# Runbook-Agent/RunbookAI

Hardware: NVIDIA H100
Metric: knn_queries_per_sec (higher is better)
Workload: dtype bf16

## Files before the change

### runbookai_b200/csrc/rbk_epilogue.cuh

```cuda
#pragma once
#include "rbk_internal.h"
#include "rbk_ptx.cuh"

namespace rbk {

struct FilterState {
  float thr;
  float inv_q;
  float qn;
  int tb;
  int mb_cache;
  int cnt;
  bool valid;
  bool nohist;
  unsigned long long* list;
  unsigned int* hist_q;
  int* maxbin_q;
};

__device__ __forceinline__ int score_bin(float a) {
  const int b = static_cast<int>((a + 1.0f) * (kHistBins * 0.5f));
  return min(max(b, 0), kHistBins - 1);
}
__device__ __forceinline__ float bin_edge_raw(int b, float qn) {
  const float edge = static_cast<float>(b) * (2.0f / kHistBins) - 1.0f - 1e-6f;
  const float r = edge * qn;
  return r - fabsf(r) * 1e-6f;
}

__device__ __forceinline__ void filter_init(FilterState& s, bool valid, float thr_init, float inv_q,
                                            unsigned long long* list, unsigned int* hist_q, int* maxbin_q) {
  s.valid = valid && thr_init < INFINITY;
  s.thr = s.valid ? thr_init : INFINITY;
  s.inv_q = s.valid ? inv_q : 0.f;
  s.qn = s.valid ? 1.0f / inv_q : 0.f;
  s.tb = (s.valid && thr_init > -INFINITY) ? score_bin(thr_init * inv_q) : -1;
  s.mb_cache = -1;
  s.nohist = false;
  s.cnt = 0;
  s.list = list;
  s.hist_q = hist_q;
  s.maxbin_q = maxbin_q;
}

static __device__ __noinline__ unsigned long long histogram_walk(const unsigned int* hist_q, int mb, int tb, float qn,
                                                                  int kprime) {
  const uint4* h4 = reinterpret_cast<const uint4*>(hist_q);
  const int g_lo = (tb + 1) >> 2;
  unsigned cum = 0;
  for (int g_hi = mb >> 2; g_hi >= g_lo; g_hi -= 4) {
    uint4 w[4];
#pragma unroll
    for (int u = 0; u < 4; ++u) w[u] = (g_hi - u >= g_lo) ? __ldcg(h4 + g_hi - u) : make_uint4(0u, 0u, 0u, 0u);
#pragma unroll
    for (int u = 0; u < 4; ++u) {
      const int g = g_hi - u;
      const unsigned c[4] = {w[u].x, w[u].y, w[u].z, w[u].w};
#pragma unroll
      for (int j = 3; j >= 0; --j) {
        const int b = g * 4 + j;
        if (g >= g_lo && b <= mb && b > tb) {
          cum += c[j];
          if (cum >= static_cast<unsigned>(kprime))
            return (static_cast<unsigned long long>(b + 1) << 32) | __float_as_uint(bin_edge_raw(b, qn));
        }
      }
    }
  }
  return 0ull;
}
__device__ __forceinline__ bool filter_refresh(FilterState& s, int kprime) {
  if (!s.valid) return false;
  const int mb = __ldcg(s.maxbin_q);
  if (mb <= s.tb) return false;
  const unsigned long long r = histogram_walk(s.hist_q, mb, s.tb, s.qn, kprime);
  if (r == 0ull) return false;
  s.tb = static_cast<int>(r >> 32) - 1;
  s.thr = fmaxf(s.thr, __uint_as_float(static_cast<uint32_t>(r)));
  return true;
}

__device__ __forceinline__ bool refresh_due(int it) {
  return it != 0 && (it < 8 || (it < 64 && (it & 7) == 0) || (it & 31) == 0);
}
__device__ __forceinline__ bool publish_due(int it) {
  return it != 0 && (it < 16 || (it < 64 && (it & 1) == 0) || (it & 7) == 0);
}
__device__ __forceinline__ void publish_threshold(FilterState& s, unsigned int* gthr_q, int kprime) {
  if (!s.valid) return;
  s.tb = max(s.tb, score_bin(s.thr * s.inv_q) - 1);
  filter_refresh(s, kprime);
  if (s.thr > -INFINITY) atomicMax(gthr_q, f32_ordered(s.thr));
}
__device__ __forceinline__ void adopt_threshold(FilterState& s, unsigned int ordered) {
  s.thr = fmaxf(s.thr, f32_from_ordered(ordered));
}

__device__ __forceinline__ void hist_add(FilterState& s, float t) {
  const int b = score_bin(t * s.inv_q);
  atomicAdd(s.hist_q + b, 1u);
  if (b > s.mb_cache) {
    atomicMax(s.maxbin_q, b);
    s.mb_cache = b;
  }
}

__device__ __forceinline__ void filter_append(FilterState& s, float t, uint32_t row) {
  s.list[s.cnt] = pack_key(t, row);
  ++s.cnt;
  if (s.nohist) return;
  hist_add(s, t);
}

__device__ __forceinline__ void seed_chunk(FilterState& s, const uint32_t (&v)[32], bool whole_tile, float& acc1,
                                           float& acc2) {
  float m1 = -INFINITY, m2 = -INFINITY;
#pragma unroll
  for (int j = 0; j < 8; ++j) {
    const float a0 = __uint_as_float(v[4 * j + 0]);
    const float a1 = __uint_as_float(v[4 * j + 1]);
    const float a2 = __uint_as_float(v[4 * j + 2]);
    const float a3 = __uint_as_float(v[4 * j + 3]);
    const float x = fmaxf(fmaxf(fmaxf(a0, a1), fmaxf(a2, a3)), -INFINITY);
    m2 = fmaxf(m2, fminf(m1, x));
    m1 = fmaxf(m1, x);
  }
  if (whole_tile) {
    const float lo = fmaxf(fminf(acc1, m1), fmaxf(acc2, m2));
    acc1 = fmaxf(acc1, m1);
    acc2 = lo;
    return;
  }
  if (m1 > s.thr) hist_add(s, m1);
  if (m2 > s.thr) hist_add(s, m2);
}

__device__ __forceinline__ void filter_chunk(FilterState& s, const uint32_t (&v)[32], uint32_t row_base) {
  float g[8];
  float m = -INFINITY;
#pragma unroll
  for (int j = 0; j < 8; ++j) {
    const float a0 = __uint_as_float(v[4 * j + 0]);
    const float a1 = __uint_as_float(v[4 * j + 1]);
    const float a2 = __uint_as_float(v[4 * j + 2]);
    const float a3 = __uint_as_float(v[4 * j + 3]);
    g[j] = fmaxf(fmaxf(a0, a1), fmaxf(a2, a3));
    m = fmaxf(m, g[j]);
  }
  if (m > s.thr) {
#pragma unroll
    for (int j = 0; j < 8; ++j) {
      if (g[j] > s.thr) {
#pragma unroll
        for (int e = 0; e < 4; ++e) {
          const float t = __uint_as_float(v[4 * j + e]);
          if (t > s.thr) filter_append(s, t, row_base + 4 * j + e);
        }
      }
    }
  }
}

__device__ __forceinline__ unsigned long long umax64(unsigned long long a, unsigned long long b) {
  return a > b ? a : b;
}
__device__ __forceinline__ unsigned long long umin64(unsigned long long a, unsigned long long b) {
  return a < b ? a : b;
}

static __device__ __noinline__ unsigned long long warp_compact(unsigned long long* list, int cnt, int kprime, int lane) {
  constexpr uint32_t kFullMask = 0xFFFFFFFFu;
  unsigned long long k[8];
#pragma unroll
  for (int j = 0; j < 8; ++j) {
    const int idx = j * 32 + lane;
    k[j] = idx < cnt ? __ldcg(list + idx) : 0ull;
  }
#pragma unroll
  for (int k2 = 2; k2 <= 256; k2 <<= 1) {
#pragma unroll
    for (int st = k2 >> 1; st > 0; st >>= 1) {
      if (st >= 32) {
        const int js = st >> 5;
#pragma unroll
        for (int j = 0; j < 8; ++j) {
          if ((j & js) == 0) {
            const int i = j * 32 + lane;
            const bool desc = (i & k2) == 0;
            const unsigned long long a = k[j], b = k[j | js];
            const unsigned long long hi = umax64(a, b), lo = umin64(a, b);
            k[j] = desc ? hi : lo;
            k[j | js] = desc ? lo : hi;
          }
        }
      } else {
#pragma unroll
        for (int j = 0; j < 8; ++j) {
          const int i = j * 32 + lane;
          const unsigned long long other = __shfl_xor_sync(kFullMask, k[j], st);
          const bool lower = (lane & st) == 0;
          const bool desc = (i & k2) == 0;
          k[j] = (lower == desc) ? umax64(k[j], other) : umin64(k[j], other);
        }
      }
    }
  }
  const int keep = cnt < kprime ? cnt : kprime;
#pragma unroll
  for (int j = 0; j < 8; ++j) {
    const int idx = j * 32 + lane;
    if (idx < keep) list[idx] = k[j];
  }
  const int e = kprime - 1;
  unsigned long long sel = 0ull;
#pragma unroll
  for (int j = 0; j < 8; ++j)
    if (j == (e >> 5)) sel = k[j];
  const unsigned long long kth = __shfl_sync(kFullMask, sel, e & 31);
  const float new_thr = cnt >= kprime ? key_score(kth) : -INFINITY;
  __syncwarp();
  return (static_cast<unsigned long long>(__float_as_uint(new_thr)) << 32) | static_cast<unsigned>(keep);
}

__device__ __forceinline__ void filter_compact_if_needed(FilterState& s, int kprime, int lane, int room = 32) {
  constexpr uint32_t kFullMask = 0xFFFFFFFFu;
  __syncwarp();
  unsigned need = __ballot_sync(kFullMask, s.cnt > kListCap - room);
  while (need) {
    const int src = __ffs(need) - 1;
    need &= need - 1;
    unsigned long long* l = reinterpret_cast<unsigned long long*>(
        __shfl_sync(kFullMask, reinterpret_cast<unsigned long long>(s.list), src));
    const int c = __shfl_sync(kFullMask, s.cnt, src);
    const unsigned long long r = warp_compact(l, c, kprime, lane);
    if (lane == src) {
      s.thr = fmaxf(s.thr, __uint_as_float(static_cast<uint32_t>(r >> 32)));
      s.cnt = static_cast<int>(static_cast<uint32_t>(r));
    }
  }
}


constexpr int kScorePitch = kBlockN + 4;

__device__ __forceinline__ void load_chunk(const float* src, uint32_t (&v)[32]) {
  const float4* s4 = reinterpret_cast<const float4*>(src);
#pragma unroll
  for (int j = 0; j < 8; ++j) {
    const float4 w = s4[j];
    v[4 * j + 0] = __float_as_uint(w.x);
    v[4 * j + 1] = __float_as_uint(w.y);
    v[4 * j + 2] = __float_as_uint(w.z);
    v[4 * j + 3] = __float_as_uint(w.w);
  }
}

struct StageHeader {
  unsigned long long mask;
  int last;
};
struct StageLink {
  const float* rows;
  const StageHeader* hdr;
  unsigned long long* full;
  unsigned long long* empty;
  volatile float* thr_pub;
};
__device__ __forceinline__ const float* stage_round(const StageLink& l, uint32_t phase, int qw, bool& last) {
  mbar_wait(smem_u32(l.full), phase);
  const unsigned long long mask = l.hdr->mask;
  last = l.hdr->last != 0;
  if (((mask >> qw) & 1ull) == 0ull) return nullptr;
  return l.rows + __popcll(mask & ((1ull << qw) - 1ull)) * kScorePitch;
}

__device__ __forceinline__ void run_epilogue(const ScanParams& p, const StageLink& sl, int qb, int r, int t0, int t1,
                                             int et, int lane) {
  const int q = qb * kBlockM + et;
  const bool q_valid = q < p.B;
  const size_t list_id = static_cast<size_t>(qb * p.R + r) * kBlockM + et;
  FilterState fs;
  filter_init(fs, q_valid, q_valid ? p.thr_init[q] : INFINITY, q_valid ? p.inv_norm_q[q] : 0.f,
              p.cand + list_id * static_cast<size_t>(kListCap),
              p.hist + static_cast<size_t>(q_valid ? q : 0) * kHistBins, p.maxbin + (q_valid ? q : 0));
  const int n_iter = t1 - t0;
  const int qw = et & 63;
  uint32_t phase = 0;
  float pub = -INFINITY;
  unsigned int* gthr_q = p.gthr + (q_valid ? q : 0);
  unsigned int ngt = 0u;
  for (int it = 0; it < n_iter; ++it) {
    const int tile = t0 + it;
    const int row0 = tile * kBlockN;
    adopt_threshold(fs, ngt);
    ngt = __ldcg(gthr_q);
    if (publish_due(it) && r == it % p.R) publish_threshold(fs, gthr_q, p.kprime);
    if (fs.thr > pub) *sl.thr_pub = pub = fs.thr;
    for (bool last = false; !last; phase ^= 1u) {
      const float* srow = stage_round(sl, phase, qw, last);
      const bool staged = srow != nullptr;
      if (__any_sync(0xFFFFFFFFu, staged)) {
        auto process = [&](uint32_t (&v)[32], int chunk) {
          filter_chunk(fs, v, static_cast<uint32_t>(row0 + chunk * 32));
          if (p.dbg_scores != nullptr && q_valid) {
#pragma unroll
            for (int j = 0; j < 32; ++j) {
              const int row = row0 + chunk * 32 + j;
              if (row < p.n_rows) p.dbg_scores[static_cast<size_t>(q) * p.n_rows + row] = __uint_as_float(v[j]);
            }
          }
        };
        uint32_t va[32], vb[32];
        if (it == 0) {
          float sa1 = -INFINITY, sa2 = -INFINITY;
          if (staged) {
#pragma unroll 1
            for (int chunk = 0; chunk < kBlockN / 32; ++chunk) {
              load_chunk(srow + chunk * 32, va);
              seed_chunk(fs, va, false, sa1, sa2);
            }
          }
          const int tries = (p.R * 16 >= 2 * p.kprime) ? 6 : 1;
          for (int t = 0; t < tries; ++t) {
            const bool found = staged && filter_refresh(fs, p.kprime);
            if (__all_sync(0xFFFFFFFFu, found || !fs.valid || !staged)) break;
            if (t + 1 < tries) __nanosleep(400);
          }
          if (staged && fs.valid && fs.thr > -INFINITY) atomicMax(gthr_q, f32_ordered(fs.thr));
          fs.nohist = staged;
        }
#pragma unroll 1
        for (int c2 = 0; c2 < kBlockN / 64; ++c2) {
          if (staged) {
            load_chunk(srow + (2 * c2) * 32, va);
            load_chunk(srow + (2 * c2 + 1) * 32, vb);
            process(va, 2 * c2);
            process(vb, 2 * c2 + 1);
          }
          filter_compact_if_needed(fs, p.kprime, lane, 64);
          if (it == 0 && staged && fs.valid && fs.thr == -INFINITY) adopt_threshold(fs, __ldcg(gthr_q));
        }
        fs.nohist = false;
      }
      mbar_arrive(smem_u32(sl.empty));
    }
    if (fs.thr > pub) *sl.thr_pub = pub = fs.thr;
  }
  p.cand_cnt[list_id] = fs.cnt;
}


__device__ __forceinline__ float count_floor_raw(int b, float qn, float delta) {
  const float edge = static_cast<float>(b) * (2.0f / kHistBins) - 1.0f - delta;
  const float r = edge * qn;
  return r - fabsf(r) * 1e-6f;
}

__device__ __forceinline__ void run_count_epilogue(const LargeScanParams& p, const StageLink& sl, int qb, int t0,
                                                   int t1, int et) {
  const int q = qb * kBlockM + et;
  const bool q_valid = q < p.B;
  FilterState fs;
  filter_init(fs, q_valid, q_valid ? p.thr_init[q] : INFINITY, q_valid ? p.inv_norm_q[q] : 0.f, nullptr,
              p.hist + static_cast<size_t>(q_valid ? q : 0) * kHistBins, p.maxbin + (q_valid ? q : 0));
  const float delta = q_valid ? static_cast<float>(2.0 * p.q_eps[q]) + 2.0f / kHistBins : 0.f;
  const int n_iter = t1 - t0;
  const int qw = et & 63;
  uint32_t phase = 0;
  float pub = -INFINITY;
  for (int it = 0; it < n_iter; ++it) {
    if (fs.valid && refresh_due(it)) {
      const int mb = __ldcg(fs.maxbin_q);
      if (mb > fs.tb) {
        const unsigned long long w = histogram_walk(fs.hist_q, mb, fs.tb, fs.qn, p.kprime);
        if (w != 0ull) {
          fs.tb = static_cast<int>(w >> 32) - 1;
          fs.thr = fmaxf(fs.thr, count_floor_raw(fs.tb, fs.qn, delta));
        }
      }
    }
    if (fs.thr > pub) *sl.thr_pub = pub = fs.thr;
    for (bool last = false; !last; phase ^= 1u) {
      const float* srow = stage_round(sl, phase, qw, last);
      if (srow != nullptr) {
#pragma unroll 1
        for (int chunk = 0; chunk < kBlockN / 32; ++chunk) {
          uint32_t v[32];
          load_chunk(srow + chunk * 32, v);
          float g[8];
          float m = -INFINITY;
#pragma unroll
          for (int j = 0; j < 8; ++j) {
            const float a0 = __uint_as_float(v[4 * j + 0]);
            const float a1 = __uint_as_float(v[4 * j + 1]);
            const float a2 = __uint_as_float(v[4 * j + 2]);
            const float a3 = __uint_as_float(v[4 * j + 3]);
            g[j] = fmaxf(fmaxf(a0, a1), fmaxf(a2, a3));
            m = fmaxf(m, g[j]);
          }
          if (m >= fs.thr) {
#pragma unroll
            for (int j = 0; j < 8; ++j) {
              if (g[j] >= fs.thr) {
#pragma unroll
                for (int e = 0; e < 4; ++e) {
                  const float a = __uint_as_float(v[4 * j + e]);
                  if (a >= fs.thr) hist_add(fs, a);
                }
              }
            }
          }
        }
      }
      mbar_arrive(smem_u32(sl.empty));
    }
  }
}

__device__ __forceinline__ void run_emit_epilogue(const LargeScanParams& p, const StageLink& sl, int qb, int t0,
                                                  int t1, int et) {
  const int q = qb * kBlockM + et;
  const bool q_valid = q < p.B;
  const float theta = q_valid ? p.thr_init[q] : INFINITY;
  const bool live = q_valid && theta < INFINITY;
  const long long seg = live ? p.emit_off[q] : 0;
  const int cap = live ? p.emit_cap[q] : 0;
  const int n_iter = t1 - t0;
  const int qw = et & 63;
  uint32_t phase = 0;
  *sl.thr_pub = theta;
  for (int it = 0; it < n_iter; ++it) {
    const int row0 = (t0 + it) * kBlockN;
    for (bool last = false; !last; phase ^= 1u) {
      const float* srow = stage_round(sl, phase, qw, last);
      if (srow != nullptr) {
#pragma unroll 1
        for (int chunk = 0; chunk < kBlockN / 32; ++chunk) {
          uint32_t v[32];
          load_chunk(srow + chunk * 32, v);
          uint32_t hits = 0u;
#pragma unroll
          for (int j = 0; j < 32; ++j) hits |= (__uint_as_float(v[j]) >= theta ? 1u : 0u) << j;
          if (hits != 0u && live) {
            int pos = atomicAdd(p.emit_cnt + q, __popc(hits));
            const int row_base = row0 + chunk * 32;
            while (hits != 0u) {
              const int j = __ffs(hits) - 1;
              hits &= hits - 1u;
              if (pos < cap) p.emit_rows[seg + pos] = row_base + j;
              ++pos;
            }
          }
        }
      }
      mbar_arrive(smem_u32(sl.empty));
    }
  }
}

static_assert(kMaxSubBatch / kBlockM <= 32, "one lane per query block");
__device__ __forceinline__ void lockstep_pace(volatile int* prog, int QB, int qb, int it, int max_lead, int lane) {
  if (QB <= 1 || (it & 1) != 0) return;
  if (lane == 0) prog[qb] = it;
  const bool peer = lane < QB && lane != qb;
  const int floor = it - max_lead;
  bool behind = peer && prog[lane] < floor;
  const long long w0 = clock64();
  while (__any_sync(0xFFFFFFFFu, behind)) {
    __nanosleep(200);
    if (__shfl_sync(0xFFFFFFFFu, clock64() - w0, 0) > (1ll << 24)) break;
    behind = peer && prog[lane] < floor;
  }
}

}
```

### runbookai_b200/csrc/rbk_ptx.cuh

```cuda
#pragma once
#include <cuda_runtime.h>
#include <stdint.h>

namespace rbk {

__device__ __forceinline__ uint32_t smem_u32(const void* p) {
  return static_cast<uint32_t>(__cvta_generic_to_shared(p));
}

__device__ __forceinline__ void mbar_init(uint32_t bar, uint32_t count) {
  asm volatile("mbarrier.init.shared::cta.b64 [%0], %1;" ::"r"(bar), "r"(count) : "memory");
}
__device__ __forceinline__ void fence_barrier_init() {
  asm volatile("fence.mbarrier_init.release.cluster;" ::: "memory");
}
__device__ __forceinline__ void mbar_arrive(uint32_t bar) {
  asm volatile("mbarrier.arrive.shared::cta.b64 _, [%0];" ::"r"(bar) : "memory");
}
__device__ __forceinline__ void mbar_arrive_expect_tx(uint32_t bar, uint32_t bytes) {
  asm volatile("mbarrier.arrive.expect_tx.shared::cta.b64 _, [%0], %1;" ::"r"(bar), "r"(bytes) : "memory");
}
__device__ __forceinline__ bool mbar_try_wait(uint32_t bar, uint32_t parity) {
  uint32_t ok;
  asm volatile(
      "{\n\t.reg .pred p;\n\t"
      "mbarrier.try_wait.parity.shared::cta.b64 p, [%1], %2;\n\t"
      "selp.u32 %0, 1, 0, p;\n\t}"
      : "=r"(ok)
      : "r"(bar), "r"(parity)
      : "memory");
  return ok != 0;
}
__device__ __forceinline__ void mbar_wait(uint32_t bar, uint32_t parity) {
  if (mbar_try_wait(bar, parity)) return;
  const long long t0 = clock64();
  uint32_t spins = 0;
  while (!mbar_try_wait(bar, parity)) {
    if (((++spins) & 0x3FFu) == 0 && (clock64() - t0) > (1ll << 31)) __trap();
  }
}

__device__ __forceinline__ void tma_prefetch_desc(const void* tmap) {
  asm volatile("prefetch.tensormap [%0];" ::"l"(reinterpret_cast<uint64_t>(tmap)) : "memory");
}
__device__ __forceinline__ void tma_load_2d(uint32_t smem_dst, const void* tmap, uint32_t bar, int32_t crd0,
                                            int32_t crd1) {
  asm volatile(
      "cp.async.bulk.tensor.2d.shared::cluster.global.mbarrier::complete_tx::bytes [%0], [%1, {%3, %4}], [%2];"
      :
      : "r"(smem_dst), "l"(reinterpret_cast<uint64_t>(tmap)), "r"(bar), "r"(crd0), "r"(crd1)
      : "memory");
}

__device__ __forceinline__ void bulk_load(uint32_t smem_dst, const void* src, uint32_t bytes, uint32_t bar) {
  asm volatile("cp.async.bulk.shared::cluster.global.mbarrier::complete_tx::bytes [%0], [%1], %2, [%3];"
               :
               : "r"(smem_dst), "l"(reinterpret_cast<uint64_t>(src)), "r"(bytes), "r"(bar)
               : "memory");
}

__device__ __forceinline__ void wgmma_fence() { asm volatile("wgmma.fence.sync.aligned;" ::: "memory"); }
__device__ __forceinline__ void wgmma_commit() { asm volatile("wgmma.commit_group.sync.aligned;" ::: "memory"); }
template <int N>
__device__ __forceinline__ void wgmma_wait(float (&d)[128]) {
  asm volatile("wgmma.wait_group.sync.aligned %0;" ::"n"(N) : "memory");
#pragma unroll
  for (int i = 0; i < 128; ++i) asm volatile("" : "+f"(d[i])::"memory");
}

__device__ __forceinline__ uint64_t make_sw128_kmajor_desc(uint32_t smem_addr) {
  uint64_t d = 0;
  d |= static_cast<uint64_t>((smem_addr & 0x3FFFFu) >> 4);
  d |= static_cast<uint64_t>(1) << 16;
  d |= static_cast<uint64_t>(1024 >> 4) << 32;
  d |= static_cast<uint64_t>(1) << 62;
  return d;
}

#define RBK_WGMMA_D128                                                                                              \
  "{%0, %1, %2, %3, %4, %5, %6, %7, %8, %9, %10, %11, %12, %13, %14, %15, "                                         \
  "%16, %17, %18, %19, %20, %21, %22, %23, %24, %25, %26, %27, %28, %29, %30, %31, "                                \
  "%32, %33, %34, %35, %36, %37, %38, %39, %40, %41, %42, %43, %44, %45, %46, %47, "                                \
  "%48, %49, %50, %51, %52, %53, %54, %55, %56, %57, %58, %59, %60, %61, %62, %63, "                                \
  "%64, %65, %66, %67, %68, %69, %70, %71, %72, %73, %74, %75, %76, %77, %78, %79, "                                \
  "%80, %81, %82, %83, %84, %85, %86, %87, %88, %89, %90, %91, %92, %93, %94, %95, "                                \
  "%96, %97, %98, %99, %100, %101, %102, %103, %104, %105, %106, %107, %108, %109, %110, %111, "                    \
  "%112, %113, %114, %115, %116, %117, %118, %119, %120, %121, %122, %123, %124, %125, %126, %127}"
#define RBK_WGMMA_D128_OUT(d)                                                                                         \
  "+f"(d[0]), "+f"(d[1]), "+f"(d[2]), "+f"(d[3]), "+f"(d[4]), "+f"(d[5]), "+f"(d[6]), "+f"(d[7]), "+f"(d[8]),      \
      "+f"(d[9]), "+f"(d[10]), "+f"(d[11]), "+f"(d[12]), "+f"(d[13]), "+f"(d[14]), "+f"(d[15]), "+f"(d[16]),         \
      "+f"(d[17]), "+f"(d[18]), "+f"(d[19]), "+f"(d[20]), "+f"(d[21]), "+f"(d[22]), "+f"(d[23]), "+f"(d[24]),        \
      "+f"(d[25]), "+f"(d[26]), "+f"(d[27]), "+f"(d[28]), "+f"(d[29]), "+f"(d[30]), "+f"(d[31]), "+f"(d[32]),        \
      "+f"(d[33]), "+f"(d[34]), "+f"(d[35]), "+f"(d[36]), "+f"(d[37]), "+f"(d[38]), "+f"(d[39]), "+f"(d[40]),        \
      "+f"(d[41]), "+f"(d[42]), "+f"(d[43]), "+f"(d[44]), "+f"(d[45]), "+f"(d[46]), "+f"(d[47]), "+f"(d[48]),        \
      "+f"(d[49]), "+f"(d[50]), "+f"(d[51]), "+f"(d[52]), "+f"(d[53]), "+f"(d[54]), "+f"(d[55]), "+f"(d[56]),        \
      "+f"(d[57]), "+f"(d[58]), "+f"(d[59]), "+f"(d[60]), "+f"(d[61]), "+f"(d[62]), "+f"(d[63]), "+f"(d[64]),        \
      "+f"(d[65]), "+f"(d[66]), "+f"(d[67]), "+f"(d[68]), "+f"(d[69]), "+f"(d[70]), "+f"(d[71]), "+f"(d[72]),        \
      "+f"(d[73]), "+f"(d[74]), "+f"(d[75]), "+f"(d[76]), "+f"(d[77]), "+f"(d[78]), "+f"(d[79]), "+f"(d[80]),        \
      "+f"(d[81]), "+f"(d[82]), "+f"(d[83]), "+f"(d[84]), "+f"(d[85]), "+f"(d[86]), "+f"(d[87]), "+f"(d[88]),        \
      "+f"(d[89]), "+f"(d[90]), "+f"(d[91]), "+f"(d[92]), "+f"(d[93]), "+f"(d[94]), "+f"(d[95]), "+f"(d[96]),        \
      "+f"(d[97]), "+f"(d[98]), "+f"(d[99]), "+f"(d[100]), "+f"(d[101]), "+f"(d[102]), "+f"(d[103]), "+f"(d[104]),   \
      "+f"(d[105]), "+f"(d[106]), "+f"(d[107]), "+f"(d[108]), "+f"(d[109]), "+f"(d[110]), "+f"(d[111]),              \
      "+f"(d[112]), "+f"(d[113]), "+f"(d[114]), "+f"(d[115]), "+f"(d[116]), "+f"(d[117]), "+f"(d[118]),              \
      "+f"(d[119]), "+f"(d[120]), "+f"(d[121]), "+f"(d[122]), "+f"(d[123]), "+f"(d[124]), "+f"(d[125]),              \
      "+f"(d[126]), "+f"(d[127])

__device__ __forceinline__ void wgmma_m64n256k16_bf16(float (&d)[128], uint64_t desc_a, uint64_t desc_b,
                                                      uint32_t accumulate) {
  asm volatile(
      "{\n\t.reg .pred p;\n\t"
      "setp.ne.b32 p, %130, 0;\n\t"
      "wgmma.mma_async.sync.aligned.m64n256k16.f32.bf16.bf16 " RBK_WGMMA_D128 ", %128, %129, p, 1, 1, 0, 0;\n\t}"
      : RBK_WGMMA_D128_OUT(d)
      : "l"(desc_a), "l"(desc_b), "r"(accumulate));
}
__device__ __forceinline__ void wgmma_m64n256k16_f16(float (&d)[128], uint64_t desc_a, uint64_t desc_b,
                                                     uint32_t accumulate) {
  asm volatile(
      "{\n\t.reg .pred p;\n\t"
      "setp.ne.b32 p, %130, 0;\n\t"
      "wgmma.mma_async.sync.aligned.m64n256k16.f32.f16.f16 " RBK_WGMMA_D128 ", %128, %129, p, 1, 1, 0, 0;\n\t}"
      : RBK_WGMMA_D128_OUT(d)
      : "l"(desc_a), "l"(desc_b), "r"(accumulate));
}

__device__ __forceinline__ bool elect_one() {
  uint32_t pred;
  asm volatile(
      "{\n\t.reg .pred p;\n\t"
      "elect.sync _|p, 0xFFFFFFFF;\n\t"
      "selp.u32 %0, 1, 0, p;\n\t}"
      : "=r"(pred));
  return pred != 0;
}

template <uint32_t N>
__device__ __forceinline__ void setmaxnreg_dec() {
  asm volatile("setmaxnreg.dec.sync.aligned.u32 %0;" ::"n"(N));
}
template <uint32_t N>
__device__ __forceinline__ void setmaxnreg_inc() {
  asm volatile("setmaxnreg.inc.sync.aligned.u32 %0;" ::"n"(N));
}
__device__ __forceinline__ void named_bar_sync(uint32_t id, uint32_t nthreads) {
  asm volatile("bar.sync %0, %1;" ::"r"(id), "r"(nthreads) : "memory");
}

__device__ __forceinline__ uint32_t f32_ordered(float f) {
  uint32_t u = __float_as_uint(f);
  return (u & 0x80000000u) ? ~u : (u | 0x80000000u);
}
__device__ __forceinline__ float f32_from_ordered(uint32_t o) {
  uint32_t u = (o & 0x80000000u) ? (o & 0x7FFFFFFFu) : ~o;
  return __uint_as_float(u);
}
__device__ __forceinline__ uint64_t pack_key(float score, uint32_t row) {
  return (static_cast<uint64_t>(f32_ordered(score)) << 32) | static_cast<uint64_t>(0xFFFFFFFFu - row);
}
__device__ __forceinline__ uint32_t key_row(uint64_t k) { return 0xFFFFFFFFu - static_cast<uint32_t>(k); }
__device__ __forceinline__ float key_score(uint64_t k) { return f32_from_ordered(static_cast<uint32_t>(k >> 32)); }

}
```

### runbookai_b200/csrc/rbk_scan.cu

```cuda
#define RBK_SCAN_F16 0
#include "rbk_scan_kernel.cuh"

namespace rbk {

cudaError_t launch_scan(const CUtensorMap& tmap_q, const CUtensorMap& tmap_c, const ScanParams& p,
                        cudaStream_t stream) {
  return launch_scan_mode<0>(tmap_q, tmap_c, p, stream);
}

cudaError_t launch_scan_large(const CUtensorMap& tmap_q, const CUtensorMap& tmap_c, const LargeScanParams& p,
                              LargeScanMode mode, cudaStream_t stream) {
  if (mode == kScanCount) return launch_scan_mode<kScanCount>(tmap_q, tmap_c, p, stream);
  return launch_scan_mode<kScanEmit>(tmap_q, tmap_c, p, stream);
}

}

#ifdef RBK_SCAN_CYCLE_STATS
extern "C" int rbk_scan_cycle_stats(unsigned long long* out) {
  constexpr int n = 3 * 2 * (rbk::kCycBuckets + 2);
  static const unsigned long long zero[n] = {};
  if (cudaDeviceSynchronize() != cudaSuccess ||
      cudaMemcpyFromSymbol(out, rbk::g_cycle_stats, sizeof(zero)) != cudaSuccess ||
      cudaMemcpyToSymbol(rbk::g_cycle_stats, zero, sizeof(zero)) != cudaSuccess)
    return -1;
  return n;
}
#endif
```

### runbookai_b200/csrc/rbk_scan_kernel.cuh

```cuda
#pragma once
#ifndef RBK_SCAN_F16
#error "define RBK_SCAN_F16 (0: bf16 operands, 1: fp16 operands) before including rbk_scan_kernel.cuh"
#endif
#if defined(RBK_SCAN_CYCLE_STATS) && !RBK_SCAN_F16
#define RBK_SCAN_PROBE 1
#else
#define RBK_SCAN_PROBE 0
#endif

#include "rbk_epilogue.cuh"
#include "rbk_internal.h"
#include "rbk_ptx.cuh"

namespace rbk {

namespace {

constexpr int kABytes = kBlockM * kBlockK * 2;
constexpr int kBBytes = kBlockN * kBlockK * 2;
constexpr int kStageBytes = kABytes + kBBytes;
constexpr int kMmaThreads = 256;
constexpr int kStagingBytes = 2 * kStageRows * kScorePitch * 4;
static_assert(kScanThreads == 128 + kMmaThreads, "warp roles");
static_assert(2 * kStageRows <= kBlockM, "a round never holds more rows than a warpgroup has queries");

struct SmemTail {
  float invc[2][2][kBlockN];
  float thr[kBlockM];
  StageHeader hdr[2];
  uint16_t wmask[2][2][4];
  unsigned long long full[kStages];
  unsigned long long empty[kStages];
  unsigned long long invc_full[2][2];
  unsigned long long st_full[2];
  unsigned long long st_empty[2];
};
constexpr size_t kScanSmemBytes = static_cast<size_t>(kStages) * kStageBytes + kStagingBytes + sizeof(SmemTail) + 1024;
static_assert(kScanSmemBytes <= 227 * 1024, "scan kernel shared memory exceeds the sm_90 per-block limit");

__device__ __forceinline__ void scan_mma(float (&d)[128], uint64_t desc_a, uint64_t desc_b, uint32_t accumulate) {
#if RBK_SCAN_F16
  wgmma_m64n256k16_f16(d, desc_a, desc_b, accumulate);
#else
  wgmma_m64n256k16_bf16(d, desc_a, desc_b, accumulate);
#endif
}

__device__ __forceinline__ void store_row(float* dst, const float (&d)[128], int h, int lane) {
  float* r = dst + 2 * (lane & 3);
#pragma unroll
  for (int j = 0; j < kBlockN / 8; ++j)
    *reinterpret_cast<float2*>(r + 8 * j) = make_float2(d[4 * j + 2 * h], d[4 * j + 2 * h + 1]);
}

__device__ __forceinline__ uint32_t quad_bits(uint32_t b) {
  b &= 0x11111111u;
  b = (b | (b >> 3)) & 0x03030303u;
  b = (b | (b >> 6)) & 0x000F000Fu;
  return (b | (b >> 12)) & 0xFFu;
}

enum CycleBucket { kCycFull, kCycMma, kCycHandoff, kCycPace, kCycTileEnd, kCycBuckets };
#if RBK_SCAN_PROBE
__device__ unsigned long long g_cycle_stats[3][2][kCycBuckets + 2];
__device__ __forceinline__ uint32_t sm_clock() {
  uint32_t c;
  asm volatile("mov.u32 %0, %%clock;" : "=r"(c)::"memory");
  return c;
}
struct CycleProbe {
  uint32_t t = 0, c[kCycBuckets] = {};
  __device__ __forceinline__ void mark() { t = sm_clock(); }
  __device__ __forceinline__ void lap(int b) {
    const uint32_t n = sm_clock();
    c[b] += n - t;
    t = n;
  }
  __device__ __forceinline__ void add_since(int b, uint32_t t0) { c[b] += sm_clock() - t0; }
  __device__ __forceinline__ static uint32_t now() { return sm_clock(); }
};
#else
struct CycleProbe {
  __device__ __forceinline__ void mark() {}
  __device__ __forceinline__ void lap(int) {}
  __device__ __forceinline__ void add_since(int, uint32_t) {}
  __device__ __forceinline__ static uint32_t now() { return 0u; }
};
#endif

template <int kMode, typename P>
__global__ void __launch_bounds__(kScanThreads, 1)
scan_kernel(const __grid_constant__ CUtensorMap tmap_q, const __grid_constant__ CUtensorMap tmap_c,
            const P p) {
  extern __shared__ uint8_t smem_raw[];
  const uint32_t raw_addr = smem_u32(smem_raw);
  uint8_t* smem = smem_raw + ((1024u - (raw_addr & 1023u)) & 1023u);
  float* staging = reinterpret_cast<float*>(smem + kStages * kStageBytes);
  SmemTail* tail = reinterpret_cast<SmemTail*>(smem + kStages * kStageBytes + kStagingBytes);
  const uint32_t smem_base = smem_u32(smem);

  const int warp = threadIdx.x >> 5;
  const int lane = threadIdx.x & 31;
  const int wgroup = warp >> 2;
  const int qb = blockIdx.x % p.QB;
  const int r = blockIdx.x / p.QB;
  const int t0 = static_cast<int>(static_cast<long long>(p.n_tiles) * r / p.R);
  const int t1 = static_cast<int>(static_cast<long long>(p.n_tiles) * (r + 1) / p.R);
  const int n_ks = p.dpad / kBlockK;

  if (threadIdx.x < kBlockM) tail->thr[threadIdx.x] = -INFINITY;
  if (threadIdx.x == 128) {
    tma_prefetch_desc(&tmap_q);
    tma_prefetch_desc(&tmap_c);
    for (int s = 0; s < kStages; ++s) {
      mbar_init(smem_u32(&tail->full[s]), 1);
      mbar_init(smem_u32(&tail->empty[s]), 2);
    }
    for (int w = 0; w < 2; ++w) {
      mbar_init(smem_u32(&tail->invc_full[w][0]), 1);
      mbar_init(smem_u32(&tail->invc_full[w][1]), 1);
      mbar_init(smem_u32(&tail->st_full[w]), 128);
      mbar_init(smem_u32(&tail->st_empty[w]), 64);
    }
    fence_barrier_init();
  }
  __syncthreads();

  constexpr uint32_t kEpiRegs = 152, kMmaRegs = 176;
  static_assert(128 * kEpiRegs + kMmaThreads * kMmaRegs <= kScanThreads * 168, "register split");
  if (wgroup == 0) {
    setmaxnreg_dec<kEpiRegs>();
    const int h = threadIdx.x >> 6;
    const StageLink sl{staging + h * kStageRows * kScorePitch, &tail->hdr[h], &tail->st_full[h], &tail->st_empty[h],
                       &tail->thr[threadIdx.x]};
    if constexpr (kMode == 0)
      run_epilogue(p, sl, qb, r, t0, t1, threadIdx.x, lane);
    else if constexpr (kMode == kScanCount)
      run_count_epilogue(p, sl, qb, t0, t1, threadIdx.x);
    else
      run_emit_epilogue(p, sl, qb, t0, t1, threadIdx.x);
    return;
  }

  setmaxnreg_inc<kMmaRegs>();
  const int wg = wgroup - 1;
  const bool leader = (threadIdx.x & 127) == 0;
  const bool producer = warp == 4;
  const int n_iter = t1 - t0;
  const int n_steps = n_iter * n_ks;
  volatile int* prog = p.progress + r * p.QB;
  CycleProbe probe;
  auto issue = [&](int j) {
    if (j >= n_steps) return;
    const int s = j % kStages;
    const int tile = t0 + j / n_ks, ks = j % n_ks;
    mbar_wait(smem_u32(&tail->empty[s]), static_cast<uint32_t>((j / kStages) & 1) ^ 1u);
    const uint32_t pace0 = CycleProbe::now();
    if (ks == 0) lockstep_pace(prog, p.QB, qb, tile - t0, p.max_lead_tiles, lane);
    probe.add_since(kCycPace, pace0);
    const uint32_t full = smem_u32(&tail->full[s]);
    const uint32_t a_dst = smem_base + s * kStageBytes;
    if (elect_one()) {
      mbar_arrive_expect_tx(full, kStageBytes);
      tma_load_2d(a_dst, &tmap_q, full, ks * kBlockK, qb * kBlockM);
      tma_load_2d(a_dst + kABytes, &tmap_c, full, ks * kBlockK, tile * kBlockN);
    }
    __syncwarp();
  };
  auto release = [&](int j) {
    if (leader) mbar_arrive(smem_u32(&tail->empty[j % kStages]));
    if (producer) issue(j + kStages);
  };
  auto load_invc = [&](int i) {
    if (!leader || i >= n_iter) return;
    const uint32_t bar = smem_u32(&tail->invc_full[wg][i & 1]);
    mbar_arrive_expect_tx(bar, kBlockN * 4);
    bulk_load(smem_u32(tail->invc[wg][i & 1]), p.inv_norm_c + static_cast<size_t>(t0 + i) * kBlockN, kBlockN * 4, bar);
  };
  if (producer)
    for (int j = 0; j < kStages; ++j) issue(j);
  load_invc(0);
  load_invc(1);
  const int qw0 = (warp & 3) * 16 + (lane >> 2);
  const int qw1 = qw0 + 8;
  const volatile float* thr = tail->thr + wg * 64;
  float* stage = staging + wg * kStageRows * kScorePitch;
  const uint32_t st_full = smem_u32(&tail->st_full[wg]), st_empty = smem_u32(&tail->st_empty[wg]);
  uint32_t rounds = 0;
  float acc[128];
#pragma unroll
  for (int i = 0; i < 128; ++i) acc[i] = 0.f;
  int j = 0;
  probe.mark();
  for (int i = 0; i < n_iter; ++i) {
    for (int ks = 0; ks < n_ks; ++ks, ++j) {
      const int s = j % kStages;
      mbar_wait(smem_u32(&tail->full[s]), static_cast<uint32_t>((j / kStages) & 1));
      probe.lap(kCycFull);
      const uint32_t st = smem_base + s * kStageBytes;
      const uint64_t adesc = make_sw128_kmajor_desc(st + wg * (64 * kBlockK * 2));
      const uint64_t bdesc = make_sw128_kmajor_desc(st + kABytes);
      wgmma_fence();
#pragma unroll
      for (int k = 0; k < kBlockK / 16; ++k)
        scan_mma(acc, adesc + static_cast<uint64_t>(2 * k), bdesc + static_cast<uint64_t>(2 * k), (ks | k) != 0 ? 1u : 0u);
      wgmma_commit();
      wgmma_wait<1>(acc);
      probe.lap(kCycMma);
      if (ks > 0) release(j - 1);
      probe.lap(kCycHandoff);
    }
    wgmma_wait<0>(acc);
    release(j - 1);

    mbar_wait(smem_u32(&tail->invc_full[wg][i & 1]), static_cast<uint32_t>((i >> 1) & 1));
    const float* invc = tail->invc[wg][i & 1] + 2 * (lane & 3);
    float m0 = -INFINITY, m1 = -INFINITY;
#pragma unroll
    for (int c = 0; c < kBlockN / 8; ++c) {
      const float2 w = *reinterpret_cast<const float2*>(invc + 8 * c);
      acc[4 * c + 0] *= w.x;
      acc[4 * c + 1] *= w.y;
      acc[4 * c + 2] *= w.x;
      acc[4 * c + 3] *= w.y;
      m0 = fmaxf(m0, fmaxf(acc[4 * c + 0], acc[4 * c + 1]));
      m1 = fmaxf(m1, fmaxf(acc[4 * c + 2], acc[4 * c + 3]));
    }
#pragma unroll
    for (int o = 1; o <= 2; o <<= 1) {
      m0 = fmaxf(m0, __shfl_xor_sync(0xFFFFFFFFu, m0, o));
      m1 = fmaxf(m1, __shfl_xor_sync(0xFFFFFFFFu, m1, o));
    }
    bool pass0, pass1;
    if constexpr (kMode == 0) {
      const bool all = i == 0 || p.dbg_scores != nullptr;
      pass0 = all || m0 > thr[qw0];
      pass1 = all || m1 > thr[qw1];
    } else {
      pass0 = m0 >= thr[qw0];
      pass1 = m1 >= thr[qw1];
    }
    const uint32_t wbits = quad_bits(__ballot_sync(0xFFFFFFFFu, pass0)) |
                           (quad_bits(__ballot_sync(0xFFFFFFFFu, pass1)) << 8);
    if (lane == 0) tail->wmask[wg][i & 1][warp & 3] = static_cast<uint16_t>(wbits);
    named_bar_sync(2 + wg, 128);
    load_invc(i + 2);
    const uint16_t* wm = tail->wmask[wg][i & 1];
    unsigned long long pending = static_cast<unsigned long long>(wm[0]) | static_cast<unsigned long long>(wm[1]) << 16 |
                                 static_cast<unsigned long long>(wm[2]) << 32 | static_cast<unsigned long long>(wm[3]) << 48;

    do {
      unsigned long long cur = pending;
      if (__popcll(pending) > kStageRows) {
        unsigned long long rest = pending;
        for (int k = 0; k < kStageRows; ++k) rest &= rest - 1ull;
        cur = pending ^ rest;
      }
      pending ^= cur;
      mbar_wait(st_empty, (rounds & 1u) ^ 1u);
      if ((cur >> qw0) & 1ull) store_row(stage + __popcll(cur & ((1ull << qw0) - 1ull)) * kScorePitch, acc, 0, lane);
      if ((cur >> qw1) & 1ull) store_row(stage + __popcll(cur & ((1ull << qw1) - 1ull)) * kScorePitch, acc, 1, lane);
      if (leader) {
        tail->hdr[wg].mask = cur;
        tail->hdr[wg].last = pending == 0ull;
      }
      mbar_arrive(st_full);
      ++rounds;
    } while (pending != 0ull);
    probe.lap(kCycTileEnd);
  }
  if (producer && lane == 0 && p.QB > 1) prog[qb] = 0x7FFFFFFF;
#if RBK_SCAN_PROBE
  if (leader) {
    for (int b = 0; b < kCycBuckets; ++b)
      atomicAdd(&g_cycle_stats[kMode][wg][b], static_cast<unsigned long long>(probe.c[b]));
    atomicAdd(&g_cycle_stats[kMode][wg][kCycBuckets], static_cast<unsigned long long>(n_iter));
    atomicAdd(&g_cycle_stats[kMode][wg][kCycBuckets + 1], 1ull);
  }
#endif
}

template <int kMode, typename P>
cudaError_t launch_scan_mode(const CUtensorMap& tmap_q, const CUtensorMap& tmap_c, const P& p, cudaStream_t stream) {
  cudaError_t e = cudaFuncSetAttribute(scan_kernel<kMode, P>, cudaFuncAttributeMaxDynamicSharedMemorySize,
                                       (int)kScanSmemBytes);
  if (e != cudaSuccess) return e;
  scan_kernel<kMode, P><<<p.QB * p.R, kScanThreads, kScanSmemBytes, stream>>>(tmap_q, tmap_c, p);
  return cudaGetLastError();
}

}
}
```

Baseline: 40100.

## Replace empty mbarriers with shared atomic release counter; last releaser issues TMA refill

The per-stage empty mbarrier and the dedicated producer warp are removed. Each warpgroup leader now bumps a shared counter with an acq_rel atomic, and whichever of the two arrives second issues the next TMA load for that stage directly. The lockstep pacing check is split so that peer progress is read earlier (peek) and the wait loop only runs when a peer is actually behind. This is meant to cut the refill handoff latency and the pacing polling overhead on the critical path, but it couples refill issue to the slower warpgroup and relies on odd/even counter parity being correct.

```diff
diff --git a/runbookai_b200/csrc/rbk_epilogue.cuh b/runbookai_b200/csrc/rbk_epilogue.cuh
--- a/runbookai_b200/csrc/rbk_epilogue.cuh
+++ b/runbookai_b200/csrc/rbk_epilogue.cuh
@@ -459,18 +459,19 @@
 }
 
 static_assert(kMaxSubBatch / kBlockM <= 32, "one lane per query block");
-__device__ __forceinline__ void lockstep_pace(volatile int* prog, int QB, int qb, int it, int max_lead, int lane) {
-  if (QB <= 1 || (it & 1) != 0) return;
+__device__ __forceinline__ void lockstep_peek(const volatile int* prog, int lane, bool peer, int& seen) {
+  if (peer) seen = prog[lane];
+}
+__device__ __forceinline__ void lockstep_pace(volatile int* prog, int qb, int it, int max_lead, int lane, bool peer,
+                                              int seen) {
   if (lane == 0) prog[qb] = it;
-  const bool peer = lane < QB && lane != qb;
   const int floor = it - max_lead;
-  bool behind = peer && prog[lane] < floor;
+  if (!__any_sync(0xFFFFFFFFu, peer && seen < floor)) return;
   const long long w0 = clock64();
-  while (__any_sync(0xFFFFFFFFu, behind)) {
+  while (__any_sync(0xFFFFFFFFu, peer && prog[lane] < floor)) {
+    if (__shfl_sync(0xFFFFFFFFu, clock64() - w0, 0) > (1ll << 24)) break;
     __nanosleep(200);
-    if (__shfl_sync(0xFFFFFFFFu, clock64() - w0, 0) > (1ll << 24)) break;
-    behind = peer && prog[lane] < floor;
-  }
-}
-
-}
+  }
+}
+
+}
diff --git a/runbookai_b200/csrc/rbk_ptx.cuh b/runbookai_b200/csrc/rbk_ptx.cuh
--- a/runbookai_b200/csrc/rbk_ptx.cuh
+++ b/runbookai_b200/csrc/rbk_ptx.cuh
@@ -38,6 +38,12 @@
   while (!mbar_try_wait(bar, parity)) {
     if (((++spins) & 0x3FFu) == 0 && (clock64() - t0) > (1ll << 31)) __trap();
   }
+}
+
+__device__ __forceinline__ uint32_t smem_inc_acq_rel(uint32_t addr) {
+  uint32_t old;
+  asm volatile("atom.acq_rel.cta.shared::cta.add.u32 %0, [%1], 1;" : "=r"(old) : "r"(addr) : "memory");
+  return old;
 }
 
 __device__ __forceinline__ void tma_prefetch_desc(const void* tmap) {
diff --git a/runbookai_b200/csrc/rbk_scan.cu b/runbookai_b200/csrc/rbk_scan.cu
--- a/runbookai_b200/csrc/rbk_scan.cu
+++ b/runbookai_b200/csrc/rbk_scan.cu
@@ -18,7 +18,7 @@
 
 #ifdef RBK_SCAN_CYCLE_STATS
 extern "C" int rbk_scan_cycle_stats(unsigned long long* out) {
-  constexpr int n = 3 * 2 * (rbk::kCycBuckets + 2);
+  constexpr int n = 3 * 2 * (rbk::kCycBuckets + rbk::kCycCounters);
   static const unsigned long long zero[n] = {};
   if (cudaDeviceSynchronize() != cudaSuccess ||
       cudaMemcpyFromSymbol(out, rbk::g_cycle_stats, sizeof(zero)) != cudaSuccess ||
diff --git a/runbookai_b200/csrc/rbk_scan_kernel.cuh b/runbookai_b200/csrc/rbk_scan_kernel.cuh
--- a/runbookai_b200/csrc/rbk_scan_kernel.cuh
+++ b/runbookai_b200/csrc/rbk_scan_kernel.cuh
@@ -30,7 +30,10 @@
   StageHeader hdr[2];
   uint16_t wmask[2][2][4];
   unsigned long long full[kStages];
-  unsigned long long empty[kStages];
+  uint32_t released[kStages];
+#if RBK_SCAN_PROBE
+  uint32_t issue_clk[kStages];
+#endif
   unsigned long long invc_full[2][2];
   unsigned long long st_full[2];
   unsigned long long st_empty[2];
@@ -60,16 +63,17 @@
   return (b | (b >> 12)) & 0xFFu;
 }
 
-enum CycleBucket { kCycFull, kCycMma, kCycHandoff, kCycPace, kCycTileEnd, kCycBuckets };
-#if RBK_SCAN_PROBE
-__device__ unsigned long long g_cycle_stats[3][2][kCycBuckets + 2];
+enum CycleBucket { kCycFull, kCycMma, kCycHandoff, kCycPace, kCycRefill, kCycTileEnd, kCycFetch, kCycBuckets };
+constexpr int kCycCounters = 4;
+#if RBK_SCAN_PROBE
+__device__ unsigned long long g_cycle_stats[3][2][kCycBuckets + kCycCounters];
 __device__ __forceinline__ uint32_t sm_clock() {
   uint32_t c;
   asm volatile("mov.u32 %0, %%clock;" : "=r"(c)::"memory");
   return c;
 }
 struct CycleProbe {
-  uint32_t t = 0, c[kCycBuckets] = {};
+  uint32_t t = 0, c[kCycBuckets] = {}, fetch_waits = 0, refills = 0;
   __device__ __forceinline__ void mark() { t = sm_clock(); }
   __device__ __forceinline__ void lap(int b) {
     const uint32_t n = sm_clock();
@@ -77,6 +81,14 @@
     t = n;
   }
   __device__ __forceinline__ void add_since(int b, uint32_t t0) { c[b] += sm_clock() - t0; }
+  __device__ __forceinline__ void refilled(uint32_t t0) {
+    add_since(kCycRefill, t0);
+    ++refills;
+  }
+  __device__ __forceinline__ void fetched(uint32_t issue_clk) {
+    add_since(kCycFetch, issue_clk);
+    ++fetch_waits;
+  }
   __device__ __forceinline__ static uint32_t now() { return sm_clock(); }
 };
 #else
@@ -84,6 +96,7 @@
   __device__ __forceinline__ void mark() {}
   __device__ __forceinline__ void lap(int) {}
   __device__ __forceinline__ void add_since(int, uint32_t) {}
+  __device__ __forceinline__ void refilled(uint32_t) {}
   __device__ __forceinline__ static uint32_t now() { return 0u; }
 };
 #endif
@@ -114,7 +127,7 @@
     tma_prefetch_desc(&tmap_c);
     for (int s = 0; s < kStages; ++s) {
       mbar_init(smem_u32(&tail->full[s]), 1);
-      mbar_init(smem_u32(&tail->empty[s]), 2);
+      tail->released[s] = 0u;
     }
     for (int w = 0; w < 2; ++w) {
       mbar_init(smem_u32(&tail->invc_full[w][0]), 1);
@@ -145,31 +158,38 @@
   setmaxnreg_inc<kMmaRegs>();
   const int wg = wgroup - 1;
   const bool leader = (threadIdx.x & 127) == 0;
-  const bool producer = warp == 4;
   const int n_iter = t1 - t0;
-  const int n_steps = n_iter * n_ks;
   volatile int* prog = p.progress + r * p.QB;
   CycleProbe probe;
-  auto issue = [&](int j) {
-    if (j >= n_steps) return;
-    const int s = j % kStages;
-    const int tile = t0 + j / n_ks, ks = j % n_ks;
-    mbar_wait(smem_u32(&tail->empty[s]), static_cast<uint32_t>((j / kStages) & 1) ^ 1u);
-    const uint32_t pace0 = CycleProbe::now();
-    if (ks == 0) lockstep_pace(prog, p.QB, qb, tile - t0, p.max_lead_tiles, lane);
-    probe.add_since(kCycPace, pace0);
+  auto issue = [&](int s, int it, int ks) {
+    const uint32_t issue0 = CycleProbe::now();
+#if RBK_SCAN_PROBE
+    tail->issue_clk[s] = issue0;
+#endif
     const uint32_t full = smem_u32(&tail->full[s]);
     const uint32_t a_dst = smem_base + s * kStageBytes;
-    if (elect_one()) {
-      mbar_arrive_expect_tx(full, kStageBytes);
-      tma_load_2d(a_dst, &tmap_q, full, ks * kBlockK, qb * kBlockM);
-      tma_load_2d(a_dst + kABytes, &tmap_c, full, ks * kBlockK, tile * kBlockN);
-    }
-    __syncwarp();
+    mbar_arrive_expect_tx(full, kStageBytes);
+    tma_load_2d(a_dst, &tmap_q, full, ks * kBlockK, qb * kBlockM);
+    tma_load_2d(a_dst + kABytes, &tmap_c, full, ks * kBlockK, (t0 + it) * kBlockN);
+    probe.refilled(issue0);
   };
-  auto release = [&](int j) {
-    if (leader) mbar_arrive(smem_u32(&tail->empty[j % kStages]));
-    if (producer) issue(j + kStages);
+  const bool pacer = warp == 4 && p.QB > 1;
+  const bool peer = lane < p.QB && lane != qb;
+  const int peek_ks = n_ks > 2 ? n_ks - 2 : 0;
+  int seen = 0x7FFFFFFF;
+  int r_it = kStages / n_ks, r_ks = kStages % n_ks;
+  auto release = [&](int s) {
+    if (pacer && r_ks == 0 && (r_it & 1) == 0 && r_it < n_iter) {
+      const uint32_t pace0 = CycleProbe::now();
+      lockstep_pace(prog, qb, r_it, p.max_lead_tiles, lane, peer, seen);
+      probe.add_since(kCycPace, pace0);
+    }
+    if (leader && (smem_inc_acq_rel(smem_u32(&tail->released[s])) & 1u) != 0u && r_it < n_iter) issue(s, r_it, r_ks);
+    if (pacer && r_ks == peek_ks && (r_it & 1) != 0) lockstep_peek(prog, lane, peer, seen);
+    if (++r_ks == n_ks) {
+      r_ks = 0;
+      ++r_it;
+    }
   };
   auto load_invc = [&](int i) {
     if (!leader || i >= n_iter) return;
@@ -177,8 +197,8 @@
     mbar_arrive_expect_tx(bar, kBlockN * 4);
     bulk_load(smem_u32(tail->invc[wg][i & 1]), p.inv_norm_c + static_cast<size_t>(t0 + i) * kBlockN, kBlockN * 4, bar);
   };
-  if (producer)
-    for (int j = 0; j < kStages; ++j) issue(j);
+  if (leader && wg == 0)
+    for (int j = 0; j < kStages && j / n_ks < n_iter; ++j) issue(j, j / n_ks, j % n_ks);
   load_invc(0);
   load_invc(1);
   const int qw0 = (warp & 3) * 16 + (lane >> 2);
@@ -195,7 +215,14 @@
   for (int i = 0; i < n_iter; ++i) {
     for (int ks = 0; ks < n_ks; ++ks, ++j) {
       const int s = j % kStages;
-      mbar_wait(smem_u32(&tail->full[s]), static_cast<uint32_t>((j / kStages) & 1));
+      const uint32_t full = smem_u32(&tail->full[s]), parity = static_cast<uint32_t>((j / kStages) & 1);
+#if RBK_SCAN_PROBE
+      const bool blocked = leader && !mbar_try_wait(full, parity);
+#endif
+      mbar_wait(full, parity);
+#if RBK_SCAN_PROBE
+      if (blocked) probe.fetched(tail->issue_clk[s]);
+#endif
       probe.lap(kCycFull);
       const uint32_t st = smem_base + s * kStageBytes;
       const uint64_t adesc = make_sw128_kmajor_desc(st + wg * (64 * kBlockK * 2));
@@ -207,11 +234,11 @@
       wgmma_commit();
       wgmma_wait<1>(acc);
       probe.lap(kCycMma);
-      if (ks > 0) release(j - 1);
+      if (ks > 0) release((j - 1) % kStages);
       probe.lap(kCycHandoff);
     }
     wgmma_wait<0>(acc);
-    release(j - 1);
+    release((j - 1) % kStages);
 
     mbar_wait(smem_u32(&tail->invc_full[wg][i & 1]), static_cast<uint32_t>((i >> 1) & 1));
     const float* invc = tail->invc[wg][i & 1] + 2 * (lane & 3);
@@ -269,13 +296,15 @@
     } while (pending != 0ull);
     probe.lap(kCycTileEnd);
   }
-  if (producer && lane == 0 && p.QB > 1) prog[qb] = 0x7FFFFFFF;
+  if (pacer && lane == 0) prog[qb] = 0x7FFFFFFF;
 #if RBK_SCAN_PROBE
   if (leader) {
     for (int b = 0; b < kCycBuckets; ++b)
       atomicAdd(&g_cycle_stats[kMode][wg][b], static_cast<unsigned long long>(probe.c[b]));
     atomicAdd(&g_cycle_stats[kMode][wg][kCycBuckets], static_cast<unsigned long long>(n_iter));
     atomicAdd(&g_cycle_stats[kMode][wg][kCycBuckets + 1], 1ull);
+    atomicAdd(&g_cycle_stats[kMode][wg][kCycBuckets + 2], static_cast<unsigned long long>(probe.fetch_waits));
+    atomicAdd(&g_cycle_stats[kMode][wg][kCycBuckets + 3], static_cast<unsigned long long>(probe.refills));
   }
 #endif
 }
```

Measured after the change: 41590 (median of 6 runs). 3.7% higher.
